# 3dlg-hcvc/tricolo

Measured on AMD Instinct MI355X. Metric: trimodal training samples/sec (32^3 voxel + 6-view), higher is better.
Workload: dtype f16 (f16 activation storage + f16 MFMA operands, fp32 accumulate; bf16x3 heads/GRU; within 1e-3 of the fp32 reference)

## Files before the change

include/tricolo_hip.h:

```cpp
#ifndef TRICOLO_HIP_H
#define TRICOLO_HIP_H
#include <stddef.h>
#include <stdint.h>

#ifdef __cplusplus
extern "C" {
#endif

#define TRI_FMT_F32 0
#define TRI_FMT_BF16 1
#define TRI_FMT_F16 2

int tri_version(void);
const char* tri_last_error(void);

typedef struct TriConvDesc {
    int B, ID, IH, IW, Cin;
    int OD, OH, OW, Cout;
    int KD, KH, KW, stride, pad_d, pad_h, pad_w;
} TriConvDesc;

int tri_conv_kpad(int ntaps, int cin_stored);
typedef struct TriPrepDesc {
    const float* w;
// ... 150 lines not shown
                        const float* mean, const float* invstd, float* dgamma, float* dbeta, float* c1, float* c2, float* c3,
                        float out_scale ,
                        void* stream);
int tri_bn_bwd_apply(const void* y, const void* g, const float* c1, const float* c2, const float* c3, const uint8_t* row_mask,
                     void* dy, long M, int C, const float* relu_scale, const float* relu_shift, const void* relu_out,
                     void* g_masked ,
                     int keep_inactive ,
                     int act_fmt, void* stream);
int tri_bn_bwd_pair_reduce(const void* ya, const void* yb, const void* g, const void* relu_out, long M, int C, float* partial_a,
                           float* partial_b, int act_fmt, void* stream);
int tri_bn_bwd_pair_finalize(const float* partial_a, const float* partial_b, int nblk, int C, int count_host, const float* gamma_a,
                             const float* mean_a, const float* invstd_a, float* buf_a, const float* gamma_b, const float* mean_b,
                             const float* invstd_b, float* buf_b, float out_scale, void* stream);
int tri_bn_bwd_pair_apply(const void* ya, const void* yb, const void* g, const void* relu_out, const float* buf_a, const float* buf_b,
                          void* dya, void* dyb, void* g_masked, long M, int C, int act_fmt, void* stream);

int tri_bn_relu_pool3d_fwd(const void* y, const float* scale, const float* shift, const uint8_t* mask, int B, int D, int C,
                           void* pooled, uint8_t* mask_out, int act_fmt, void* stream);
int tri_pool3d_bwd_route_rows(const void* y, const float* scale, const float* shift, const uint8_t* mask, const void* pooled,
                              const void* dpooled, int B, int D, int C, void* g, const int* out_pos, const int* out_count, int act_fmt,
                              void* stream);
int tri_pool3d_bwd_route_rows_num_blocks(int B, int D, int C);
int tri_pool3d_bwd_route_rows_reduce(const void* y, const float* scale, const float* shift, const uint8_t* mask, const void* pooled,
                                     const void* dpooled, int B, int D, int C, void* g, const int* out_pos, const int* out_count,
                                     float* partial, int act_fmt, void* stream);
int tri_bn_bwd_apply_rows(const void* y, const void* g, const float* c1, const float* c2, const float* c3, void* dy, int C,
                          const int* row_pos, const int* row_count, long max_rows, int act_fmt, void* stream);
size_t tri_bn_bwd_rows_scratch(int C);
int tri_bn_bwd_rows(const void* y, const void* g, int C, const int* row_pos, const int* row_count, long max_rows, const float* gamma,
                    const float* mean, const float* invstd, void* dy, float* dgamma, float* dbeta, float out_scale, void* scratch,
// ... 141 lines not shown
```

tricolo_amd/_C.py:

```python
from __future__ import annotations

import ctypes as C
import os

import torch

_HERE = os.path.dirname(os.path.abspath(__file__))
LIB_PATH = os.path.join(_HERE, "libtricolo_hip.so")


class TriConvDesc(C.Structure):
    _fields_ = [(n, C.c_int) for n in ("B", "ID", "IH", "IW", "Cin", "OD", "OH", "OW", "Cout",
                                       "KD", "KH", "KW", "stride", "pad_d", "pad_h", "pad_w")]


class TriPrepDesc(C.Structure):
    _fields_ = [("w", C.c_void_p), ("hi", C.c_void_p), ("lo", C.c_void_p), ("s_row", C.c_long), ("s_tap", C.c_long),
                ("s_inner", C.c_long), ("rows", C.c_int), ("ntaps", C.c_int), ("inner", C.c_int), ("inner_pad", C.c_int),
                ("kpad", C.c_int), ("fmt", C.c_int), ("frag", C.c_int)]


class TriWgradReduce(C.Structure):
    _fields_ = [("slab", C.c_void_p), ("dw", C.c_void_p), ("s_co", C.c_long), ("s_tap", C.c_long), ("s_ci", C.c_long)] + \
               [(n, C.c_int) for n in ("splits", "Cout", "Kpad", "ntaps", "cin_stored", "cin_real", "zlanes", "nblocks")] + \
# ... 57 lines not shown
    "tri_conv_stem_wgrad_bn": (I, [DP, P, P, P, P, P, P, P, P, P, P, Z, P, L, L, L, I, I, F, P, P]),
    "tri_conv_wgrad_group_info": (I, [DP, I, P, P, P]),
    "tri_conv_wgrad_partial_group": (I, [P, I, I, P, P]),
    "tri_bn_finalize": (I, [P, I, I, P, I, P, P, P, P, P, F, F, P, P, P, P, P]),
    "tri_bn_eval_coeffs": (I, [I, P, P, P, P, F, P, P, P, P, P]),
    "tri_bn_act": (I, [P, P, P, P, P, P, P, L, I, I, I, P]),
    "tri_relu_bwd": (I, [P, P, P, L, I, P]),
    "tri_bn_bwd_num_blocks": (I, [L]),
    "tri_bn_bwd_reduce": (I, [P, P, L, I, P, P, P, P, P, I, P]),
    "tri_bn_bwd_finalize": (I, [P, I, I, P, I, P, P, P, P, P, P, P, P, F, P]),
    "tri_bn_bwd_small": (I, [P, P, L, I, P, I, P, P, P, P, P, P, P, P, I, P, P, P, F, I, P]),
    "tri_bn_bwd_apply": (I, [P, P, P, P, P, P, P, L, I, P, P, P, P, I, I, P]),
    "tri_bn_bwd_pair_reduce": (I, [P, P, P, P, L, I, P, P, I, P]),
    "tri_bn_bwd_pair_finalize": (I, [P, P, I, I, I, P, P, P, P, P, P, P, P, F, P]),
    "tri_bn_bwd_pair_apply": (I, [P, P, P, P, P, P, P, P, P, L, I, I, P]),
    "tri_bn_relu_pool3d_fwd": (I, [P, P, P, P, I, I, I, P, P, I, P]),
    "tri_pool3d_bwd_route": (I, [P, P, P, P, P, P, I, I, I, P, I, P]),
    "tri_pool3d_bwd_route_rows": (I, [P, P, P, P, P, P, I, I, I, P, P, P, I, P]),
    "tri_pool3d_bwd_route_rows_num_blocks": (I, [I, I, I]),
    "tri_pool3d_bwd_route_rows_reduce": (I, [P, P, P, P, P, P, I, I, I, P, P, P, P, I, P]),
    "tri_bn_bwd_apply_rows": (I, [P, P, P, P, P, P, I, P, P, L, I, P]),
    "tri_bn_bwd_rows_scratch": (C.c_size_t, [I]),
    "tri_bn_bwd_rows": (I, [P, P, I, P, P, L, P, P, P, P, P, P, F, P, I, P]),
    "tri_pool3d_bwd_route_reduce_num_blocks": (I, [I, I, I]),
    "tri_pool3d_bwd_route_reduce": (I, [P, P, P, P, P, P, I, I, I, P, P, I, P]),
    "tri_maxpool2d_fwd": (I, [P, I, I, I, I, P, P, P, P, I, P]),
    "tri_maxpool2d_bwd": (I, [P, P, I, I, I, I, P, I, P]),
    "tri_maxpool_bn_bwd_num_blocks": (I, [I, I, I]),
    "tri_maxpool_bn_bwd_reduce": (I, [P, P, P, I, I, I, I, P, P, P, I, P]),
    "tri_maxpool_bn_bwd_pooled_num_blocks": (I, [I, I, I]),
# ... 138 lines not shown
```

tricolo_amd/csrc/bn_pool.hip:

```cpp
#include "common.h"
#include "../../include/tricolo_hip.h"

__global__ void bn_finalize_kernel(const float* __restrict__ partial, int ntiles, int C, const int* __restrict__ count_dev,
                                   int count_host, const float* __restrict__ gamma, const float* __restrict__ beta,
                                   float* running_mean, float* running_var, long long* num_batches_tracked, float momentum,
                                   float eps, float* __restrict__ mean_out, float* __restrict__ invstd_out,
                                   float* __restrict__ scale_out, float* __restrict__ shift_out) {
    __shared__ double ssum[4], ssq[4];
    const int c = blockIdx.x;
    float pg = 0.f, pb = 0.f, prm = 0.f, prv = 0.f;
    int pcount = count_host;
    if (threadIdx.x == 0) {
        pg = gamma[c]; pb = beta[c];
        if (running_mean) { prm = running_mean[c]; prv = running_var[c]; }
        if (count_dev) pcount = *count_dev;
    }
    double s = 0.0, q = 0.0;
#pragma unroll 8
    for (int tIdx = threadIdx.x; tIdx < ntiles; tIdx += 256) {
        s += (double)partial[((size_t)tIdx * 2 + 0) * C + c];
        q += (double)partial[((size_t)tIdx * 2 + 1) * C + c];
    }
#pragma unroll
    for (int o = 32; o > 0; o >>= 1) { s += __shfl_xor(s, o); q += __shfl_xor(q, o); }
// ... 162 lines not shown
    if (relu_scale && relu_out) { tri_set_error("tri_bn_bwd_reduce: give either relu_scale/shift or relu_out"); return TRI_ERR_ARG; }
#define TRI_BNR(MASK_)                                                                                                              \
    do {                                                                                                                            \
        if (row_mask) TRI_ACT_DISPATCH(act_fmt, bn_bwd_reduce_kernel<T, MASK_, true><<<nblk, 256, smem, (hipStream_t)stream>>>(       \
            (const T*)y, (const T*)g, M, C, partial, rows, (const float4*)relu_scale, (const float4*)relu_shift, (const T*)relu_out, row_mask)); \
        else TRI_ACT_DISPATCH(act_fmt, bn_bwd_reduce_kernel<T, MASK_, false><<<nblk, 256, smem, (hipStream_t)stream>>>(               \
            (const T*)y, (const T*)g, M, C, partial, rows, (const float4*)relu_scale, (const float4*)relu_shift, (const T*)relu_out, row_mask)); \
    } while (0)
    if (relu_out) TRI_BNR(2);
    else if (relu_scale) TRI_BNR(1);
    else TRI_BNR(0);
#undef TRI_BNR
    return tri_check_launch("tri_bn_bwd_reduce");
}

__device__ __forceinline__ void bn_bwd_finalize_body(const float* __restrict__ partial, int nblk, int C, const int* __restrict__ count_dev,
                                                     int count_host, const float* __restrict__ gamma, const float* __restrict__ mean,
                                                     const float* __restrict__ invstd, float* __restrict__ dgamma, float* __restrict__ dbeta,
                                                     float* __restrict__ c1, float* __restrict__ c2, float* __restrict__ c3, float out_scale,
                                                     int c) {
    __shared__ double ssum[4], ssq[4];
    float pmu = 0.f, pis = 0.f, pga = 0.f;
    int pcount = count_host;
    if (threadIdx.x == 0) {
        pmu = mean[c]; pis = invstd[c]; pga = gamma[c];
        if (count_dev) pcount = *count_dev;
    }
    double s = 0.0, q = 0.0;
#pragma unroll 8
    for (int b = threadIdx.x; b < nblk; b += 256) {
        s += (double)partial[((size_t)b * 2 + 0) * C + c];
        q += (double)partial[((size_t)b * 2 + 1) * C + c];
    }
#pragma unroll
    for (int o = 32; o > 0; o >>= 1) { s += __shfl_xor(s, o); q += __shfl_xor(q, o); }
    if ((threadIdx.x & 63) == 0) { ssum[threadIdx.x >> 6] = s; ssq[threadIdx.x >> 6] = q; }
    __syncthreads();
    if (threadIdx.x == 0) {
        s = (ssum[0] + ssum[1]) + (ssum[2] + ssum[3]);
        q = (ssq[0] + ssq[1]) + (ssq[2] + ssq[3]);
        double n = (double)pcount;
        if (n < 1.0) { dgamma[c] = 0.f; dbeta[c] = 0.f; c1[c] = 0.f; c2[c] = 0.f; c3[c] = 0.f; return; }
        double mu = pmu, is = pis, ga = pga;
        double dbe = s;
        double dga = is * (q - mu * s);
        dgamma[c] = (float)(dga * (double)out_scale);
        dbeta[c] = (float)(dbe * (double)out_scale);
        double k1 = ga * is;
        double k3 = -ga * is * is * dga / n;
        double k2 = -k1 * dbe / n - k3 * mu;
        c1[c] = (float)k1; c2[c] = (float)k2; c3[c] = (float)k3;
    }
}
__global__ void bn_bwd_finalize_kernel(const float* __restrict__ partial, int nblk, int C, const int* __restrict__ count_dev,
                                       int count_host, const float* __restrict__ gamma, const float* __restrict__ mean,
                                       const float* __restrict__ invstd, float* __restrict__ dgamma, float* __restrict__ dbeta,
                                       float* __restrict__ c1, float* __restrict__ c2, float* __restrict__ c3, float out_scale) {
    bn_bwd_finalize_body(partial, nblk, C, count_dev, count_host, gamma, mean, invstd, dgamma, dbeta, c1, c2, c3, out_scale, blockIdx.x);
}
__global__ void bn_bwd_finalize_pair_kernel(const float* __restrict__ pa, const float* __restrict__ pb, int nblk, int C, int count_host,
                                            const float* __restrict__ ga, const float* __restrict__ ma, const float* __restrict__ ia,
                                            float* __restrict__ buf_a, const float* __restrict__ gb, const float* __restrict__ mb,
                                            const float* __restrict__ ib, float* __restrict__ buf_b, float out_scale) {
    const bool second = (int)blockIdx.x >= C;
    const int c = second ? blockIdx.x - C : blockIdx.x;
    float* buf = second ? buf_b : buf_a;
// ... 139 lines not shown
                                        const float* invstd_b, float* buf_b, float out_scale, void* stream) {
    bn_bwd_finalize_pair_kernel<<<2 * C, 256, 0, (hipStream_t)stream>>>(partial_a, partial_b, nblk, C, count_host, gamma_a, mean_a, invstd_a, buf_a,
                                                                       gamma_b, mean_b, invstd_b, buf_b, out_scale);
    return tri_check_launch("tri_bn_bwd_pair_finalize");
}
extern "C" int tri_bn_bwd_pair_apply(const void* ya, const void* yb, const void* g, const void* relu_out, const float* buf_a, const float* buf_b,
                                     void* dya, void* dyb, void* g_masked, long M, int C, int act_fmt, void* stream) {
    if (C % 4) { tri_set_error("tri_bn_bwd_pair_apply: C must be a multiple of 4"); return TRI_ERR_ARG; }
    const long total4 = M * (C / 4);
    TRI_ACT_DISPATCH(act_fmt, bn_bwd_apply_pair_kernel<T><<<ew_grid(total4), 256, 0, (hipStream_t)stream>>>(
        (const T*)ya, (const T*)yb, (const T*)g, (const float4*)(buf_a + 2 * C), (const float4*)(buf_b + 2 * C), (T*)dya, (T*)dyb, total4, C / 4,
        (const T*)relu_out, (T*)g_masked));
    return tri_check_launch("tri_bn_bwd_pair_apply");
}

template <typename T, int MASK, int CH>
__global__ __launch_bounds__(256) void bn_bwd_small_kernel(const T* __restrict__ y, const T* g, long M, int C, const int* __restrict__ count_dev,
                                                           int count_host, const float* __restrict__ gamma, const float* __restrict__ mean,
                                                           const float* __restrict__ invstd, const float* __restrict__ rs,
                                                           const float* __restrict__ rb, const T* __restrict__ ro, T* gm,
                                                           const uint8_t* __restrict__ row_mask, int keep_inactive, T* dy,
                                                           float* __restrict__ dgamma, float* __restrict__ dbeta, float out_scale) {
    constexpr int Q = CH / 4;
    __shared__ float red[4][2 * CH];
    __shared__ float coef[3 * CH];
    const int nblk = gridDim.x;
    const int grp = (nblk % 8 == 0) ? (int)(blockIdx.x % 8) * (nblk / 8) + (int)(blockIdx.x / 8) : (int)blockIdx.x;
    const int c0 = grp * CH;
    const int t = threadIdx.x;
    float4 s4[Q], b4[Q];
// ... 1015 lines not shown
```

tricolo_amd/model/module/img_encoder/mv_cnn.py:

```python
from __future__ import annotations

import contextlib
import os

import torch
import torch.nn as nn

from .... import ops
from ....layers import SideStream, TriModule, linear_bwd, linear_fwd, require_gpu


_DS_FWD = int(os.environ.get("TRICOLO_DS_FWD", "2"))
_DS_BWD = int(os.environ.get("TRICOLO_DS_BWD", "2"))
_PREP_DGRAD_LATE = os.environ.get("TRICOLO_PREP_DGRAD_LATE", "1") != "0"
_BN_PAIR = True
_STEM_BESIDE_WGRAD = os.environ.get("TRICOLO_STEM_BESIDE_WGRAD", "1") != "0"
_PREP_ISSUE = int(os.environ.get("TRICOLO_PREP_ISSUE", "1"))


class _BasicBlockParams(nn.Module):
    def __init__(self, inplanes, planes, stride):
        super().__init__()
        self.conv1 = nn.Conv2d(inplanes, planes, 3, stride, 1, bias=False)
        self.bn1 = nn.BatchNorm2d(planes)
# ... 261 lines not shown
                gr[w] = ops.conv_wgrad(x, dy, g, w, prec, out_scale=ugs, batch=batch)
                return
            with torch.cuda.stream(side.fork(x, dy)):
                gr[w] = ops.conv_wgrad(x, dy, g, w, prec, out_scale=ugs)

        dout_sums = None
        for bi in range(len(blocks) - 1, -1, -1):
            blk, sv = blocks[bi], saved_blocks[bi]
            x, y1, co1, g1, a1, y2, co2, g2, yd, cod, gd, out = sv
            pair = (_BN_PAIR and blk.downsample is not None and batch is not None and dout_sums is None and yd is not None
                    and yd.shape == y2.shape and ops._sync_world() == 1)
            dyd_pair = None
            if pair:
                (dy2, gr[blk.bn2.weight], gr[blk.bn2.bias], dyd_pair, gr[blk.downsample[1].weight],
                 gr[blk.downsample[1].bias]) = ops.bn_bwd_pair(y2, co2, blk.bn2.weight, yd, cod, blk.downsample[1].weight, dout, out, g2.M,
                                                               g_masked=dout, out_scale=ugs)
            else:
                dy2, gr[blk.bn2.weight], gr[blk.bn2.bias] = ops.bn_bwd(y2, dout, co2, blk.bn2.weight, count_host=g2.M, inplace=False,
                                                                       relu_out=out, g_masked=dout, out_scale=ugs, partial=dout_sums)
            g = dout
            fine = ops.TIMELINE is not None and ops.TIMELINE.get("fine")
            tag = f"image.bwd.c{y2.shape[-1]}.b{bi}"
            if fine:
                ops.stamp(tag + ".bn2")
            mode = _DS_BWD if (blk.downsample is not None and batch is not None) else 0
            ev = None
            if mode == 2:
                ev = torch.cuda.Event()
                ev.record()

            def shortcut_bwd():
                with torch.cuda.stream(self._side_ds.fork(g, yd, event=ev)):
                    if dyd_pair is not None:
                        return dyd_pair, ops.conv_dgrad(dyd_pair, gd, self._packed[(id(blk.downsample[0]), True)])
                    dyd_, gr[blk.downsample[1].weight], gr[blk.downsample[1].bias] = ops.bn_bwd(
                        yd, g, cod, blk.downsample[1].weight, count_host=gd.M, inplace=False, out_scale=ugs)
                    if batch is None:
                        gr[blk.downsample[0].weight] = ops.conv_wgrad(x, dyd_, gd, blk.downsample[0].weight, prec, out_scale=ugs)
                    return dyd_, ops.conv_dgrad(dyd_, gd, self._packed[(id(blk.downsample[0]), True)])
            if blk.downsample is not None and not mode:
                dyd, dx = shortcut_bwd()
            wgrad_async(a1, dy2, g2, blk.conv2.weight)
            da1, sums1 = ops.conv_dgrad(dy2, g2, self._packed[(id(blk.conv2), True)], bn_sums=(y1, co1, None))
            if mode:
                dyd, dx = shortcut_bwd()
            if fine:
                ops.stamp(tag + ".dgrad2")
            dy1, gr[blk.bn1.weight], gr[blk.bn1.bias] = ops.bn_bwd(y1, da1, co1, blk.bn1.weight, count_host=g1.M, relu=True, out_scale=ugs,
                                                                   partial=sums1)
            if fine:
                ops.stamp(tag + ".bn1")
            wgrad_async(x, dy1, g1, blk.conv1.weight)
            if blk.downsample is not None:
                if batch is None:
                    self._side_ds.join(dx, gr[blk.downsample[0].weight], gr[blk.downsample[1].weight], gr[blk.downsample[1].bias])
                else:
                    self._side_ds.join(dx, dyd, gr[blk.downsample[1].weight], gr[blk.downsample[1].bias])
                    gr[blk.downsample[0].weight] = ops.conv_wgrad(x, dyd, gd, blk.downsample[0].weight, prec, out_scale=ugs, batch=batch)
            else:
                dx = g
            if bi > 0:
                prev = saved_blocks[bi - 1]
                dx, dout_sums = ops.conv_dgrad(dy1, g1, self._packed[(id(blk.conv1), True)], out=dx, accumulate=True,
                                               bn_sums=(prev[5], None, prev[11]))
# ... 122 lines not shown
```

tricolo_amd/ops.py:

```python
from __future__ import annotations

import collections
import math
import os

import torch

from . import _C
from ._C import check, lib, make_desc, ptr, stream

_PRECISIONS = ("bf16", "bf16x3", "f16")
_FMT = {torch.float32: 0, torch.bfloat16: 1, torch.float16: 2}
F16_GRAD_SCALE = float(os.environ.get("TRICOLO_F16_GRAD_SCALE", "4096"))
if not (F16_GRAD_SCALE >= 1.0 and math.frexp(F16_GRAD_SCALE)[0] == 0.5):
    raise ValueError(f"TRICOLO_F16_GRAD_SCALE={F16_GRAD_SCALE!r}: must be a power of two >= 1 (the kernels divide it out exactly)")
_default_precision = os.environ.get("TRICOLO_PRECISION", "bf16x3")


def set_default_precision(p: str):
    global _default_precision
    if p not in _PRECISIONS:
        raise ValueError(f"precision must be one of {_PRECISIONS}")
    _default_precision = p

# ... 660 lines not shown
        tot = _sync_sum(partial.sum(0, keepdim=True).contiguous())
        if count_dev is not None:
            count_dev = _sync_sum(count_dev.clone())
        else:
            count_host = int(count_host) * world
        gbuf = torch.empty((5, C), dtype=torch.float32, device=partial.device)
        check(lib().tri_bn_bwd_finalize(ptr(tot), 1, C, ptr(count_dev), int(count_host), ptr(gamma), ptr(co.mean), ptr(co.invstd), ptr(gbuf[0]),
                                        ptr(gbuf[1]), ptr(gbuf[2]), ptr(gbuf[3]), ptr(gbuf[4]), float(out_scale), stream()), "tri_bn_bwd_finalize")
        buf = torch.stack([buf[0], buf[1], gbuf[2], gbuf[3], gbuf[4]])
    return buf


_BN_SMALL = True


def _bn_bwd_finish(y, g, partial, co: BNCoeffs, gamma, count_dev, count_host, out_scale, dy, row_mask=None, keep_inactive=False, rows=None,
                   rs=None, rb=None, relu_out=None, g_masked=None):
    C = y.shape[-1]
    buf = _bn_bwd_finalize(partial, partial.shape[0], C, count_dev, count_host, gamma, co, out_scale)
    if rows is not None:
        check(lib().tri_bn_bwd_apply_rows(ptr(y), ptr(g), ptr(buf[2]), ptr(buf[3]), ptr(buf[4]), ptr(dy), C, ptr(rows[0]), ptr(rows[1]),
                                          rows[0].numel(), _abf(y), stream()), "tri_bn_bwd_apply_rows")
    else:
        check(lib().tri_bn_bwd_apply(ptr(y), ptr(g), ptr(buf[2]), ptr(buf[3]), ptr(buf[4]), ptr(row_mask), ptr(dy), y.numel() // C, C, ptr(rs), ptr(rb),
                                     ptr(relu_out), ptr(g_masked), 1 if keep_inactive else 0, _abf(y), stream()), "tri_bn_bwd_apply")
    return dy, buf[0], buf[1]


def bn_bwd(y, g, co: BNCoeffs, gamma, count_dev=None, count_host=0, row_mask=None, inplace=True, relu=False, relu_out=None,
           g_masked=None, out_scale: float = 1.0, keep_inactive: bool = False, partial=None):
    rs, rb = (co.scale, co.shift) if relu else (None, None)
    C = y.shape[-1]
    M = y.numel() // C
    assert y.dtype == g.dtype
    dy = g if inplace else torch.empty_like(g)
    if partial is None and _BN_SMALL and M <= 512 and C % 8 == 0 and C >= 64 and _sync_world() == 1:
        buf = torch.empty((2, C), dtype=torch.float32, device=y.device)
        check(lib().tri_bn_bwd_small(ptr(_act(y)), ptr(_act(g)), M, C, ptr(count_dev), int(count_host), ptr(gamma), ptr(co.mean), ptr(co.invstd),
                                     ptr(rs), ptr(rb), ptr(relu_out), ptr(g_masked), ptr(row_mask), 1 if keep_inactive else 0, ptr(dy), ptr(buf[0]),
                                     ptr(buf[1]), float(out_scale), _abf(y), stream()), "tri_bn_bwd_small")
        return dy, buf[0], buf[1]
    if partial is None:
        partial = torch.empty((lib().tri_bn_bwd_num_blocks(M), 2, C), dtype=torch.float32, device=y.device)
        check(lib().tri_bn_bwd_reduce(ptr(_act(y)), ptr(_act(g)), M, C, ptr(partial), ptr(rs), ptr(rb), ptr(relu_out), ptr(row_mask), _abf(y), stream()),
              "tri_bn_bwd_reduce")
    assert partial.shape[1:] == (2, C)
    return _bn_bwd_finish(y, g, partial, co, gamma, count_dev, count_host, out_scale, dy, row_mask=row_mask, keep_inactive=keep_inactive,
                          rs=rs, rb=rb, relu_out=relu_out, g_masked=g_masked)


def bn_bwd_pair(ya, coa: BNCoeffs, gamma_a, yb, cob: BNCoeffs, gamma_b, g, relu_out, count_host, g_masked=None, out_scale: float = 1.0):
    C = ya.shape[-1]
    M = ya.numel() // C
    assert ya.dtype == g.dtype == yb.dtype == relu_out.dtype and ya.shape == yb.shape and _sync_world() == 1
    nblk = lib().tri_bn_bwd_num_blocks(M)
    partial = torch.empty((2, nblk, 2, C), dtype=torch.float32, device=ya.device)
    check(lib().tri_bn_bwd_pair_reduce(ptr(_act(ya)), ptr(_act(yb)), ptr(_act(g)), ptr(relu_out), M, C, ptr(partial[0]), ptr(partial[1]), _abf(ya),
                                       stream()), "tri_bn_bwd_pair_reduce")
    buf = torch.empty((2, 5, C), dtype=torch.float32, device=ya.device)
    check(lib().tri_bn_bwd_pair_finalize(ptr(partial[0]), ptr(partial[1]), nblk, C, int(count_host), ptr(gamma_a), ptr(coa.mean), ptr(coa.invstd),
                                         ptr(buf[0]), ptr(gamma_b), ptr(cob.mean), ptr(cob.invstd), ptr(buf[1]), float(out_scale), stream()),
          "tri_bn_bwd_pair_finalize")
    dya, dyb = torch.empty_like(ya), torch.empty_like(yb)
    check(lib().tri_bn_bwd_pair_apply(ptr(ya), ptr(yb), ptr(g), ptr(relu_out), ptr(buf[0]), ptr(buf[1]), ptr(dya), ptr(dyb), ptr(g_masked), M, C,
                                      _abf(ya), stream()), "tri_bn_bwd_pair_apply")
    return dya, buf[0, 0], buf[0, 1], dyb, buf[1, 0], buf[1, 1]


def bn_relu_pool3d_fwd(y, co: BNCoeffs, mask, B, D, C, want_mask: bool = True):
# ... 957 lines not shown
```

Baseline: 13150.

## Fuse BN backward finalize into apply for a two-launch path in image encoder

Adds a two-launch BN backward path. A column-tiled reduce (centred on a bf16-rounded mean) is followed by an apply kernel that rebuilds the per-channel coefficients from the partial records in every workgroup, so the separate finalize launch goes away. The image encoder's residual blocks opt into it for the pair, single and relu-masked BN backward calls when M is at most 16384. Each apply workgroup now re-reduces up to 192 records, which adds redundant work in exchange for one fewer launch and no finalize round trip.

```diff
diff --git a/include/tricolo_hip.h b/include/tricolo_hip.h
--- a/include/tricolo_hip.h
+++ b/include/tricolo_hip.h
@@ -188,6 +188,21 @@
                              const float* invstd_b, float* buf_b, float out_scale, void* stream);
 int tri_bn_bwd_pair_apply(const void* ya, const void* yb, const void* g, const void* relu_out, const float* buf_a, const float* buf_b,
                           void* dya, void* dyb, void* g_masked, long M, int C, int act_fmt, void* stream);
+int tri_bnbwd2_records(long M, int C);
+int tri_bnbwd2_max_records(void);
+int tri_bnbwd2_reduce(const void* y, const void* g, long M, int C, float* partial, const float* relu_scale, const float* relu_shift,
+                      const void* relu_out, const float* mean , int act_fmt, void* stream);
+int tri_bnbwd2_apply(const void* y, const void* g, const float* partial, int nrec,
+                     int centred ,
+                     long M, int C, int count_host, const float* gamma, const float* mean, const float* invstd, float* dgamma, float* dbeta,
+                     float out_scale, const float* relu_scale, const float* relu_shift, const void* relu_out, void* g_masked, void* dy,
+                     int act_fmt, void* stream);
+int tri_bnbwd2_pair_reduce(const void* ya, const void* yb, const void* g, const void* relu_out, long M, int C, float* partial_a,
+                           float* partial_b, const float* mean_a, const float* mean_b, int act_fmt, void* stream);
+int tri_bnbwd2_pair_apply(const void* ya, const void* yb, const void* g, const void* relu_out, const float* partial_a,
+                          const float* partial_b, int nrec, long M, int C, int count_host, const float* gamma_a, const float* mean_a,
+                          const float* invstd_a, float* buf_a, const float* gamma_b, const float* mean_b, const float* invstd_b,
+                          float* buf_b, float out_scale, void* dya, void* dyb, void* g_masked, int act_fmt, void* stream);
 
 int tri_bn_relu_pool3d_fwd(const void* y, const float* scale, const float* shift, const uint8_t* mask, int B, int D, int C,
                            void* pooled, uint8_t* mask_out, int act_fmt, void* stream);
diff --git a/tricolo_amd/_C.py b/tricolo_amd/_C.py
--- a/tricolo_amd/_C.py
+++ b/tricolo_amd/_C.py
@@ -95,6 +95,12 @@
     "tri_bn_bwd_pair_reduce": (I, [P, P, P, P, L, I, P, P, I, P]),
     "tri_bn_bwd_pair_finalize": (I, [P, P, I, I, I, P, P, P, P, P, P, P, P, F, P]),
     "tri_bn_bwd_pair_apply": (I, [P, P, P, P, P, P, P, P, P, L, I, I, P]),
+    "tri_bnbwd2_records": (I, [L, I]),
+    "tri_bnbwd2_max_records": (I, []),
+    "tri_bnbwd2_reduce": (I, [P, P, L, I, P, P, P, P, P, I, P]),
+    "tri_bnbwd2_apply": (I, [P, P, P, I, I, L, I, I, P, P, P, P, P, F, P, P, P, P, P, I, P]),
+    "tri_bnbwd2_pair_reduce": (I, [P, P, P, P, L, I, P, P, P, P, I, P]),
+    "tri_bnbwd2_pair_apply": (I, [P, P, P, P, P, P, I, L, I, I, P, P, P, P, P, P, P, P, F, P, P, P, I, P]),
     "tri_bn_relu_pool3d_fwd": (I, [P, P, P, P, I, I, I, P, P, I, P]),
     "tri_pool3d_bwd_route": (I, [P, P, P, P, P, P, I, I, I, P, I, P]),
     "tri_pool3d_bwd_route_rows": (I, [P, P, P, P, P, P, I, I, I, P, P, P, I, P]),
diff --git a/tricolo_amd/csrc/bn_pool.hip b/tricolo_amd/csrc/bn_pool.hip
--- a/tricolo_amd/csrc/bn_pool.hip
+++ b/tricolo_amd/csrc/bn_pool.hip
@@ -200,6 +200,19 @@
     return tri_check_launch("tri_bn_bwd_reduce");
 }
 
+struct BnBwdCoeffs { float dgamma, dbeta, c1, c2, c3; };
+__device__ __forceinline__ BnBwdCoeffs bn_bwd_coeffs(double s, double q, double n, double mu, double is, double ga, float out_scale) {
+    BnBwdCoeffs r;
+    double dbe = s;
+    double dga = is * (q - mu * s);
+    r.dgamma = (float)(dga * (double)out_scale);
+    r.dbeta = (float)(dbe * (double)out_scale);
+    double k1 = ga * is;
+    double k3 = -ga * is * is * dga / n;
+    double k2 = -k1 * dbe / n - k3 * mu;
+    r.c1 = (float)k1; r.c2 = (float)k2; r.c3 = (float)k3;
+    return r;
+}
 __device__ __forceinline__ void bn_bwd_finalize_body(const float* __restrict__ partial, int nblk, int C, const int* __restrict__ count_dev,
                                                      int count_host, const float* __restrict__ gamma, const float* __restrict__ mean,
                                                      const float* __restrict__ invstd, float* __restrict__ dgamma, float* __restrict__ dbeta,
@@ -227,15 +240,9 @@
         q = (ssq[0] + ssq[1]) + (ssq[2] + ssq[3]);
         double n = (double)pcount;
         if (n < 1.0) { dgamma[c] = 0.f; dbeta[c] = 0.f; c1[c] = 0.f; c2[c] = 0.f; c3[c] = 0.f; return; }
-        double mu = pmu, is = pis, ga = pga;
-        double dbe = s;
-        double dga = is * (q - mu * s);
-        dgamma[c] = (float)(dga * (double)out_scale);
-        dbeta[c] = (float)(dbe * (double)out_scale);
-        double k1 = ga * is;
-        double k3 = -ga * is * is * dga / n;
-        double k2 = -k1 * dbe / n - k3 * mu;
-        c1[c] = (float)k1; c2[c] = (float)k2; c3[c] = (float)k3;
+        const BnBwdCoeffs k = bn_bwd_coeffs(s, q, n, pmu, pis, pga, out_scale);
+        dgamma[c] = k.dgamma; dbeta[c] = k.dbeta;
+        c1[c] = k.c1; c2[c] = k.c2; c3[c] = k.c3;
     }
 }
 __global__ void bn_bwd_finalize_kernel(const float* __restrict__ partial, int nblk, int C, const int* __restrict__ count_dev,
@@ -405,6 +412,308 @@
     return tri_check_launch("tri_bn_bwd_pair_apply");
 }
 
+static const int BN2_CH = 64;
+static const int BN2_RECORDS = 192;
+static const int BN2_APPLY_WGS = 768;
+struct Bn2Plan { long rows; int chunks; };
+static inline Bn2Plan bn2_plan(long M, int C, int wgs) {
+    long want = wgs / (C / BN2_CH);
+    if (want < 1) want = 1;
+    long rows = ((M + want - 1) / want + 15) / 16 * 16;
+    if (rows < 16) rows = 16;
+    Bn2Plan p;
+    p.rows = rows; p.chunks = (int)((M + rows - 1) / rows);
+    return p;
+}
+static int bn2_args_ok(long M, int C) {
+    if (M < 1 || C < BN2_CH || C % BN2_CH) { tri_set_error("tri_bnbwd2_*: needs M >= 1 rows and C a multiple of 64"); return 0; }
+    return 1;
+}
+template <int MASK>
+__device__ __forceinline__ float4 bn2_masked(float4 gv, const float4& yv, const float4& s4, const float4& b4, const float4& ov) {
+    if (MASK == 1) {
+        gv.x = __fmaf_rn(yv.x, s4.x, b4.x) > 0.f ? gv.x : 0.f; gv.y = __fmaf_rn(yv.y, s4.y, b4.y) > 0.f ? gv.y : 0.f;
+        gv.z = __fmaf_rn(yv.z, s4.z, b4.z) > 0.f ? gv.z : 0.f; gv.w = __fmaf_rn(yv.w, s4.w, b4.w) > 0.f ? gv.w : 0.f;
+    }
+    if (MASK == 2) { gv.x = ov.x > 0.f ? gv.x : 0.f; gv.y = ov.y > 0.f ? gv.y : 0.f; gv.z = ov.z > 0.f ? gv.z : 0.f; gv.w = ov.w > 0.f ? gv.w : 0.f; }
+    return gv;
+}
+__device__ __forceinline__ double bn2_sum16(const double* v) {
+    return (((v[0] + v[1]) + (v[2] + v[3])) + ((v[4] + v[5]) + (v[6] + v[7]))) + (((v[8] + v[9]) + (v[10] + v[11])) + ((v[12] + v[13]) + (v[14] + v[15])));
+}
+__device__ __forceinline__ float bn2_centre(float mean) { return (float)(bf16_t)mean; }
+template <typename T, int MASK>
+__global__ __launch_bounds__(256) void bn2_reduce_kernel(const T* __restrict__ y, const T* __restrict__ g, long M, int C, float* __restrict__ partial,
+                                                         long rows, const float4* __restrict__ rs, const float4* __restrict__ rb,
+                                                         const T* __restrict__ ro, const float4* __restrict__ mu) {
+    __shared__ double sh[16][16][8];
+    const int tc = threadIdx.x & 15, tr = threadIdx.x >> 4;
+    const int c4 = blockIdx.y * 16 + tc;
+    const long r0 = (long)blockIdx.x * rows;
+    const long r1 = r0 + rows < M ? r0 + rows : M;
+    double a[8] = {0, 0, 0, 0, 0, 0, 0, 0};
+    float4 s4 = make_float4(0, 0, 0, 0), b4 = make_float4(1, 1, 1, 1);
+    if (MASK == 1) { s4 = rs[c4]; b4 = rb[c4]; }
+    float4 m4 = make_float4(0, 0, 0, 0);
+    if (mu) { m4 = mu[c4]; m4 = make_float4(bn2_centre(m4.x), bn2_centre(m4.y), bn2_centre(m4.z), bn2_centre(m4.w)); }
+#pragma unroll 8
+    for (long r = r0 + tr; r < r1; r += 16) {
+        const long o = r * C + c4 * 4;
+        const float4 yv = Act<T>::ld4(y + o);
+        float4 ov = make_float4(0, 0, 0, 0);
+        if (MASK == 2) ov = Act<T>::ld4(ro + o);
+        const float4 gv = bn2_masked<MASK>(Act<T>::ld4(g + o), yv, s4, b4, ov);
+        a[0] += (double)gv.x; a[1] += (double)gv.y; a[2] += (double)gv.z; a[3] += (double)gv.w;
+        a[4] = fma((double)gv.x, (double)yv.x - (double)m4.x, a[4]); a[5] = fma((double)gv.y, (double)yv.y - (double)m4.y, a[5]);
+        a[6] = fma((double)gv.z, (double)yv.z - (double)m4.z, a[6]); a[7] = fma((double)gv.w, (double)yv.w - (double)m4.w, a[7]);
+    }
+    double* p = sh[tr][tc];
+#pragma unroll
+    for (int k = 0; k < 8; ++k) p[k] = a[k];
+    __syncthreads();
+    if (threadIdx.x < 128) {
+        const int half = threadIdx.x >> 6, ch = threadIdx.x & 63;
+        double v[16];
+#pragma unroll
+        for (int rr = 0; rr < 16; ++rr) v[rr] = sh[rr][ch >> 2][half * 4 + (ch & 3)];
+        partial[((size_t)blockIdx.x * 2 + half) * C + blockIdx.y * BN2_CH + ch] = (float)bn2_sum16(v);
+    }
+}
+__device__ __forceinline__ void bn2_coeffs(const float* __restrict__ partial, int nrec, int C, int c0, int count_host,
+                                           const float* __restrict__ gamma, const float* __restrict__ mean, const float* __restrict__ invstd,
+                                           float out_scale, bool centred, bool write, float* __restrict__ dgamma, float* __restrict__ dbeta,
+                                           double (*red)[128], float* coef) {
+    const int t = threadIdx.x;
+    float pmu = 0.f, pis = 0.f, pga = 0.f;
+    if (t < BN2_CH) { pmu = mean[c0 + t]; pis = invstd[c0 + t]; pga = gamma[c0 + t]; }
+    const int q = t & 31, lane = t >> 5;
+    const float* p = partial + (size_t)(q >> 4) * C + c0 + (q & 15) * 4;
+    double s0 = 0.0, s1 = 0.0, s2 = 0.0, s3 = 0.0;
+#pragma unroll 8
+    for (int b = lane; b < nrec; b += 8) {
+        const float4 v = *(const float4*)(p + (size_t)b * 2 * C);
+        s0 += (double)v.x; s1 += (double)v.y; s2 += (double)v.z; s3 += (double)v.w;
+    }
+    red[lane][q * 4 + 0] = s0; red[lane][q * 4 + 1] = s1; red[lane][q * 4 + 2] = s2; red[lane][q * 4 + 3] = s3;
+    __syncthreads();
+    if (t < BN2_CH) {
+        const double s = ((red[0][t] + red[1][t]) + (red[2][t] + red[3][t])) + ((red[4][t] + red[5][t]) + (red[6][t] + red[7][t]));
+        double sq = ((red[0][64 + t] + red[1][64 + t]) + (red[2][64 + t] + red[3][64 + t])) +
+                    ((red[4][64 + t] + red[5][64 + t]) + (red[6][64 + t] + red[7][64 + t]));
+        if (centred) sq = fma((double)bn2_centre(pmu), s, sq);
+        const double n = (double)count_host;
+        BnBwdCoeffs k = {0.f, 0.f, 0.f, 0.f, 0.f};
+        if (n >= 1.0) k = bn_bwd_coeffs(s, sq, n, pmu, pis, pga, out_scale);
+        coef[t] = k.c1; coef[BN2_CH + t] = k.c2; coef[2 * BN2_CH + t] = k.c3;
+        if (write) { dgamma[c0 + t] = k.dgamma; dbeta[c0 + t] = k.dbeta; }
+    }
+    __syncthreads();
+}
+template <typename T>
+__device__ __forceinline__ void bn2_store_twice(T* p, const float4& d, const float4& y, const float4& t) {
+    float4 o;
+    o.x = fp32_rounded(__fmaf_rn(d.x, y.x, t.x)); o.y = fp32_rounded(__fmaf_rn(d.y, y.y, t.y));
+    o.z = fp32_rounded(__fmaf_rn(d.z, y.z, t.z)); o.w = fp32_rounded(__fmaf_rn(d.w, y.w, t.w));
+    Act<T>::st4(p, o);
+}
+template <typename T>
+__device__ __forceinline__ void bn2_store_once(T* p, const float4& d, const float4& y, const float4& t) { bn2_store_twice(p, d, y, t); }
+template <>
+__device__ __forceinline__ void bn2_store_once<f16_t>(f16_t* p, const float4& d, const float4& y, const float4& t) {
+#if defined(__HIP_DEVICE_COMPILE__)
+    uint2 w = make_uint2(0u, 0u);
+    asm("v_fma_mixlo_f16 %0, %1, %2, %3 op_sel_hi:[0,0,0]" : "+v"(w.x) : "v"(d.x), "v"(y.x), "v"(t.x));
+    asm("v_fma_mixhi_f16 %0, %1, %2, %3 op_sel_hi:[0,0,0]" : "+v"(w.x) : "v"(d.y), "v"(y.y), "v"(t.y));
+    asm("v_fma_mixlo_f16 %0, %1, %2, %3 op_sel_hi:[0,0,0]" : "+v"(w.y) : "v"(d.z), "v"(y.z), "v"(t.z));
+    asm("v_fma_mixhi_f16 %0, %1, %2, %3 op_sel_hi:[0,0,0]" : "+v"(w.y) : "v"(d.w), "v"(y.w), "v"(t.w));
+    *(uint2*)p = w;
+#endif
+}
+__device__ __forceinline__ float4 bn2_fma4(const float4& a, const float4& g, const float4& b) {
+    return make_float4(__fmaf_rn(a.x, g.x, b.x), __fmaf_rn(a.y, g.y, b.y), __fmaf_rn(a.z, g.z, b.z), __fmaf_rn(a.w, g.w, b.w));
+}
+static const int BN2_U = 4;
+template <typename T, int MASK>
+__global__ __launch_bounds__(256) void bn2_apply_kernel(const T* __restrict__ y, const T* g, const float* __restrict__ partial, int nrec, long M,
+                                                        int C, int count_host, const float* __restrict__ gamma, const float* __restrict__ mean,
+                                                        const float* __restrict__ invstd, float* __restrict__ dgamma, float* __restrict__ dbeta,
+                                                        float out_scale, int centred, long rows, const float4* __restrict__ rs,
+                                                        const float4* __restrict__ rb, const T* __restrict__ ro, T* gm, T* dy) {
+    __shared__ double red[8][128];
+    __shared__ __attribute__((aligned(16))) float coef[3 * BN2_CH];
+    const int c0 = blockIdx.y * BN2_CH;
+    const int tc = threadIdx.x & 15, tr = threadIdx.x >> 4;
+    float4 s4 = make_float4(0, 0, 0, 0), b4 = make_float4(1, 1, 1, 1);
+    if (MASK == 1) { s4 = rs[c0 / 4 + tc]; b4 = rb[c0 / 4 + tc]; }
+    bn2_coeffs(partial, nrec, C, c0, count_host, gamma, mean, invstd, out_scale, centred != 0, blockIdx.x == 0, dgamma, dbeta, red, coef);
+    const float4 a = ((const float4*)coef)[tc], b = ((const float4*)(coef + BN2_CH))[tc], d = ((const float4*)(coef + 2 * BN2_CH))[tc];
+    const long r0 = (long)blockIdx.x * rows;
+    const long r1 = r0 + rows < M ? r0 + rows : M;
+    for (long r = r0 + tr; r < r1; r += 16 * BN2_U) {
+        float4 yv[BN2_U], gv[BN2_U], ov[BN2_U];
+#pragma unroll
+        for (int u = 0; u < BN2_U; ++u) {
+            const long o = (r + 16 * u) * C + c0 + tc * 4;
+            ov[u] = make_float4(0, 0, 0, 0);
+            if (r + 16 * u < r1) {
+                yv[u] = Act<T>::ld4(y + o); gv[u] = Act<T>::ld4(g + o);
+                if (MASK == 2) ov[u] = Act<T>::ld4(ro + o);
+            }
+        }
+#pragma unroll
+        for (int u = 0; u < BN2_U; ++u) {
+            if (r + 16 * u >= r1) continue;
+            const long o = (r + 16 * u) * C + c0 + tc * 4;
+            const float4 gm4 = bn2_masked<MASK>(gv[u], yv[u], s4, b4, ov[u]);
+            if (MASK == 2 && gm) Act<T>::st4(gm + o, gm4);
+            if (MASK == 0) bn2_store_once(dy + o, d, yv[u], bn2_fma4(a, gm4, b));
+            else bn2_store_twice(dy + o, d, yv[u], bn2_fma4(a, gm4, b));
+        }
+    }
+}
+template <typename T>
+__global__ __launch_bounds__(256) void bn2_reduce_pair_kernel(const T* __restrict__ ya, const T* __restrict__ yb, const T* __restrict__ g, long M,
+                                                              int C, float* __restrict__ partial_a, float* __restrict__ partial_b, long rows,
+                                                              const T* __restrict__ ro, const float4* __restrict__ mua,
+                                                              const float4* __restrict__ mub) {
+    __shared__ double sh[16][16][12];
+    const int tc = threadIdx.x & 15, tr = threadIdx.x >> 4;
+    const int c4 = blockIdx.y * 16 + tc;
+    const long r0 = (long)blockIdx.x * rows;
+    const long r1 = r0 + rows < M ? r0 + rows : M;
+    double a[12] = {0, 0, 0, 0, 0, 0, 0, 0, 0, 0, 0, 0};
+    float4 ma = mua[c4], mb = mub[c4];
+    ma = make_float4(bn2_centre(ma.x), bn2_centre(ma.y), bn2_centre(ma.z), bn2_centre(ma.w));
+    mb = make_float4(bn2_centre(mb.x), bn2_centre(mb.y), bn2_centre(mb.z), bn2_centre(mb.w));
+#pragma unroll 4
+    for (long r = r0 + tr; r < r1; r += 16) {
+        const long o = r * C + c4 * 4;
+        float4 gv = Act<T>::ld4(g + o);
+        const float4 av = Act<T>::ld4(ya + o), bv = Act<T>::ld4(yb + o), ov = Act<T>::ld4(ro + o);
+        gv.x = ov.x > 0.f ? gv.x : 0.f; gv.y = ov.y > 0.f ? gv.y : 0.f; gv.z = ov.z > 0.f ? gv.z : 0.f; gv.w = ov.w > 0.f ? gv.w : 0.f;
+        a[0] += (double)gv.x; a[1] += (double)gv.y; a[2] += (double)gv.z; a[3] += (double)gv.w;
+        a[4] = fma((double)gv.x, (double)av.x - (double)ma.x, a[4]); a[5] = fma((double)gv.y, (double)av.y - (double)ma.y, a[5]);
+        a[6] = fma((double)gv.z, (double)av.z - (double)ma.z, a[6]); a[7] = fma((double)gv.w, (double)av.w - (double)ma.w, a[7]);
+        a[8] = fma((double)gv.x, (double)bv.x - (double)mb.x, a[8]); a[9] = fma((double)gv.y, (double)bv.y - (double)mb.y, a[9]);
+        a[10] = fma((double)gv.z, (double)bv.z - (double)mb.z, a[10]); a[11] = fma((double)gv.w, (double)bv.w - (double)mb.w, a[11]);
+    }
+    double* p = sh[tr][tc];
+#pragma unroll
+    for (int k = 0; k < 12; ++k) p[k] = a[k];
+    __syncthreads();
+    if (threadIdx.x < 192) {
+        const int which = threadIdx.x >> 6, ch = threadIdx.x & 63;
+        double v[16];
+#pragma unroll
+        for (int rr = 0; rr < 16; ++rr) v[rr] = sh[rr][ch >> 2][which * 4 + (ch & 3)];
+        const float a = (float)bn2_sum16(v);
+        const size_t rec = (size_t)blockIdx.x * 2 * C + blockIdx.y * BN2_CH + ch;
+        if (which == 0) { partial_a[rec] = a; partial_b[rec] = a; }
+        else if (which == 1) partial_a[rec + C] = a;
+        else partial_b[rec + C] = a;
+    }
+}
+template <typename T>
+__global__ __launch_bounds__(256) void bn2_apply_pair_kernel(const T* __restrict__ ya, const T* __restrict__ yb, const T* g,
+                                                             const float* __restrict__ partial_a, const float* __restrict__ partial_b, int nrec,
+                                                             long M, int C, int count_host, const float* __restrict__ ga,
+                                                             const float* __restrict__ ma, const float* __restrict__ ia, float* __restrict__ buf_a,
+                                                             const float* __restrict__ gb, const float* __restrict__ mb,
+                                                             const float* __restrict__ ib, float* __restrict__ buf_b, float out_scale, long rows,
+                                                             const T* __restrict__ ro, T* gm, T* dya, T* dyb) {
+    __shared__ double red[8][128];
+    __shared__ __attribute__((aligned(16))) float coef[2][3 * BN2_CH];
+    const int c0 = blockIdx.y * BN2_CH;
+    const int tc = threadIdx.x & 15, tr = threadIdx.x >> 4;
+    bn2_coeffs(partial_a, nrec, C, c0, count_host, ga, ma, ia, out_scale, true, blockIdx.x == 0, buf_a, buf_a + C, red, coef[0]);
+    bn2_coeffs(partial_b, nrec, C, c0, count_host, gb, mb, ib, out_scale, true, blockIdx.x == 0, buf_b, buf_b + C, red, coef[1]);
+    const float4 a1 = ((const float4*)coef[0])[tc], a2 = ((const float4*)(coef[0] + BN2_CH))[tc], a3 = ((const float4*)(coef[0] + 2 * BN2_CH))[tc];
+    const float4 b1 = ((const float4*)coef[1])[tc], b2 = ((const float4*)(coef[1] + BN2_CH))[tc], b3 = ((const float4*)(coef[1] + 2 * BN2_CH))[tc];
+    const long r0 = (long)blockIdx.x * rows;
+    const long r1 = r0 + rows < M ? r0 + rows : M;
+    constexpr int U = 2;
+    for (long r = r0 + tr; r < r1; r += 16 * U) {
+        float4 av[U], bv[U], gv[U], ov[U];
+#pragma unroll
+        for (int u = 0; u < U; ++u) {
+            const long o = (r + 16 * u) * C + c0 + tc * 4;
+            if (r + 16 * u < r1) { gv[u] = Act<T>::ld4(g + o); av[u] = Act<T>::ld4(ya + o); bv[u] = Act<T>::ld4(yb + o); ov[u] = Act<T>::ld4(ro + o); }
+        }
+#pragma unroll
+        for (int u = 0; u < U; ++u) {
+            if (r + 16 * u >= r1) continue;
+            const long o = (r + 16 * u) * C + c0 + tc * 4;
+            float4 m = gv[u];
+            m.x = ov[u].x > 0.f ? m.x : 0.f; m.y = ov[u].y > 0.f ? m.y : 0.f; m.z = ov[u].z > 0.f ? m.z : 0.f; m.w = ov[u].w > 0.f ? m.w : 0.f;
+            if (gm) Act<T>::st4(gm + o, m);
+            bn2_store_twice(dya + o, a3, av[u], bn2_fma4(a1, m, a2));
+            bn2_store_once(dyb + o, b3, bv[u], bn2_fma4(b1, m, b2));
+        }
+    }
+}
+extern "C" int tri_bnbwd2_records(long M, int C) {
+    if (M < 1 || C < BN2_CH || C % BN2_CH) return 0;
+    return bn2_plan(M, C, BN2_RECORDS).chunks;
+}
+extern "C" int tri_bnbwd2_max_records(void) { return BN2_RECORDS; }
+extern "C" int tri_bnbwd2_reduce(const void* y, const void* g, long M, int C, float* partial, const float* relu_scale, const float* relu_shift,
+                                 const void* relu_out, const float* mean, int act_fmt, void* stream) {
+    if (!bn2_args_ok(M, C)) return TRI_ERR_UNSUPPORTED;
+    if ((relu_scale && relu_out) || (!relu_scale != !relu_shift)) { tri_set_error("tri_bnbwd2_reduce: give relu_scale + relu_shift, or relu_out, or neither"); return TRI_ERR_ARG; }
+    const Bn2Plan pl = bn2_plan(M, C, BN2_RECORDS);
+    const dim3 grid(pl.chunks, C / BN2_CH);
+#define TRI_BN2R(MASK_)                                                                                                                 \
+    TRI_ACT_DISPATCH(act_fmt, bn2_reduce_kernel<T, MASK_><<<grid, 256, 0, (hipStream_t)stream>>>(                                      \
+        (const T*)y, (const T*)g, M, C, partial, pl.rows, (const float4*)relu_scale, (const float4*)relu_shift, (const T*)relu_out,  \
+        (const float4*)mean))
+    if (relu_out) TRI_BN2R(2);
+    else if (relu_scale) TRI_BN2R(1);
+    else TRI_BN2R(0);
+#undef TRI_BN2R
+    return tri_check_launch("tri_bnbwd2_reduce");
+}
+extern "C" int tri_bnbwd2_apply(const void* y, const void* g, const float* partial, int nrec, int centred, long M, int C, int count_host,
+                                const float* gamma, const float* mean, const float* invstd, float* dgamma, float* dbeta, float out_scale, const float* relu_scale,
+                                const float* relu_shift, const void* relu_out, void* g_masked, void* dy, int act_fmt, void* stream) {
+    if (!bn2_args_ok(M, C)) return TRI_ERR_UNSUPPORTED;
+    if (nrec < 1 || nrec > BN2_RECORDS) { tri_set_error("tri_bnbwd2_apply: 1 .. 192 records"); return TRI_ERR_UNSUPPORTED; }
+    if ((relu_scale && relu_out) || (!relu_scale != !relu_shift)) { tri_set_error("tri_bnbwd2_apply: give relu_scale + relu_shift, or relu_out, or neither"); return TRI_ERR_ARG; }
+    const Bn2Plan pl = bn2_plan(M, C, BN2_APPLY_WGS);
+    const dim3 grid(pl.chunks, C / BN2_CH);
+#define TRI_BN2A(MASK_)                                                                                                                 \
+    TRI_ACT_DISPATCH(act_fmt, bn2_apply_kernel<T, MASK_><<<grid, 256, 0, (hipStream_t)stream>>>(                                       \
+        (const T*)y, (const T*)g, partial, nrec, M, C, count_host, gamma, mean, invstd, dgamma, dbeta, out_scale, centred, pl.rows,     \
+        (const float4*)relu_scale, (const float4*)relu_shift, (const T*)relu_out, (T*)g_masked, (T*)dy))
+    if (relu_out) TRI_BN2A(2);
+    else if (relu_scale) TRI_BN2A(1);
+    else TRI_BN2A(0);
+#undef TRI_BN2A
+    return tri_check_launch("tri_bnbwd2_apply");
+}
+extern "C" int tri_bnbwd2_pair_reduce(const void* ya, const void* yb, const void* g, const void* relu_out, long M, int C, float* partial_a,
+                                      float* partial_b, const float* mean_a, const float* mean_b, int act_fmt, void* stream) {
+    if (!bn2_args_ok(M, C)) return TRI_ERR_UNSUPPORTED;
+    if (!relu_out || !mean_a || !mean_b) { tri_set_error("tri_bnbwd2_pair_reduce: the saved output and both means are required"); return TRI_ERR_ARG; }
+    const Bn2Plan pl = bn2_plan(M, C, BN2_RECORDS);
+    const dim3 grid(pl.chunks, C / BN2_CH);
+    TRI_ACT_DISPATCH(act_fmt, bn2_reduce_pair_kernel<T><<<grid, 256, 0, (hipStream_t)stream>>>(
+        (const T*)ya, (const T*)yb, (const T*)g, M, C, partial_a, partial_b, pl.rows, (const T*)relu_out, (const float4*)mean_a, (const float4*)mean_b));
+    return tri_check_launch("tri_bnbwd2_pair_reduce");
+}
+extern "C" int tri_bnbwd2_pair_apply(const void* ya, const void* yb, const void* g, const void* relu_out, const float* partial_a,
+                                     const float* partial_b, int nrec, long M, int C, int count_host, const float* gamma_a, const float* mean_a,
+                                     const float* invstd_a, float* buf_a, const float* gamma_b, const float* mean_b, const float* invstd_b,
+                                     float* buf_b, float out_scale, void* dya, void* dyb, void* g_masked, int act_fmt, void* stream) {
+    if (!bn2_args_ok(M, C)) return TRI_ERR_UNSUPPORTED;
+    if (nrec < 1 || nrec > BN2_RECORDS || !relu_out) { tri_set_error("tri_bnbwd2_pair_apply: 1 .. 192 records and the saved output"); return TRI_ERR_UNSUPPORTED; }
+    const Bn2Plan pl = bn2_plan(M, C, BN2_APPLY_WGS);
+    const dim3 grid(pl.chunks, C / BN2_CH);
+    TRI_ACT_DISPATCH(act_fmt, bn2_apply_pair_kernel<T><<<grid, 256, 0, (hipStream_t)stream>>>(
+        (const T*)ya, (const T*)yb, (const T*)g, partial_a, partial_b, nrec, M, C, count_host, gamma_a, mean_a, invstd_a, buf_a, gamma_b, mean_b,
+        invstd_b, buf_b, out_scale, pl.rows, (const T*)relu_out, (T*)g_masked, (T*)dya, (T*)dyb));
+    return tri_check_launch("tri_bnbwd2_pair_apply");
+}
+
 template <typename T, int MASK, int CH>
 __global__ __launch_bounds__(256) void bn_bwd_small_kernel(const T* __restrict__ y, const T* g, long M, int C, const int* __restrict__ count_dev,
                                                            int count_host, const float* __restrict__ gamma, const float* __restrict__ mean,
diff --git a/tricolo_amd/model/module/img_encoder/mv_cnn.py b/tricolo_amd/model/module/img_encoder/mv_cnn.py
--- a/tricolo_amd/model/module/img_encoder/mv_cnn.py
+++ b/tricolo_amd/model/module/img_encoder/mv_cnn.py
@@ -299,10 +299,10 @@
             if pair:
                 (dy2, gr[blk.bn2.weight], gr[blk.bn2.bias], dyd_pair, gr[blk.downsample[1].weight],
                  gr[blk.downsample[1].bias]) = ops.bn_bwd_pair(y2, co2, blk.bn2.weight, yd, cod, blk.downsample[1].weight, dout, out, g2.M,
-                                                               g_masked=dout, out_scale=ugs)
+                                                               g_masked=dout, out_scale=ugs, two_launch=True)
             else:
                 dy2, gr[blk.bn2.weight], gr[blk.bn2.bias] = ops.bn_bwd(y2, dout, co2, blk.bn2.weight, count_host=g2.M, inplace=False,
-                                                                       relu_out=out, g_masked=dout, out_scale=ugs, partial=dout_sums)
+                                                                       relu_out=out, g_masked=dout, out_scale=ugs, partial=dout_sums, two_launch=True)
             g = dout
             fine = ops.TIMELINE is not None and ops.TIMELINE.get("fine")
             tag = f"image.bwd.c{y2.shape[-1]}.b{bi}"
@@ -332,7 +332,7 @@
             if fine:
                 ops.stamp(tag + ".dgrad2")
             dy1, gr[blk.bn1.weight], gr[blk.bn1.bias] = ops.bn_bwd(y1, da1, co1, blk.bn1.weight, count_host=g1.M, relu=True, out_scale=ugs,
-                                                                   partial=sums1)
+                                                                   partial=sums1, two_launch=True)
             if fine:
                 ops.stamp(tag + ".bn1")
             wgrad_async(x, dy1, g1, blk.conv1.weight)
diff --git a/tricolo_amd/ops.py b/tricolo_amd/ops.py
--- a/tricolo_amd/ops.py
+++ b/tricolo_amd/ops.py
@@ -698,9 +698,24 @@
 _BN_SMALL = True
 
 
+_BN2_MAX_ROWS = 16384
+
+
+def _bn_bwd_two_launches(asked, M, C, nrec=None, count_dev=None, row_mask=None, rows=None) -> bool:
+    if not asked or row_mask is not None or rows is not None or count_dev is not None or C % 64 or M > _BN2_MAX_ROWS or _sync_world() != 1:
+        return False
+    return nrec is None or 1 <= nrec <= lib().tri_bnbwd2_max_records()
+
+
 def _bn_bwd_finish(y, g, partial, co: BNCoeffs, gamma, count_dev, count_host, out_scale, dy, row_mask=None, keep_inactive=False, rows=None,
-                   rs=None, rb=None, relu_out=None, g_masked=None):
+                   rs=None, rb=None, relu_out=None, g_masked=None, two_launch=False, centred=False):
     C = y.shape[-1]
+    if _bn_bwd_two_launches(two_launch, y.numel() // C, C, partial.shape[0], count_dev, row_mask, rows):
+        buf = torch.empty((2, C), dtype=torch.float32, device=partial.device)
+        check(lib().tri_bnbwd2_apply(ptr(y), ptr(g), ptr(partial), partial.shape[0], 1 if centred else 0, y.numel() // C, C, int(count_host), ptr(gamma), ptr(co.mean),
+                                     ptr(co.invstd), ptr(buf[0]), ptr(buf[1]), float(out_scale), ptr(rs), ptr(rb), ptr(relu_out), ptr(g_masked),
+                                     ptr(dy), _abf(y), stream()), "tri_bnbwd2_apply")
+        return dy, buf[0], buf[1]
     buf = _bn_bwd_finalize(partial, partial.shape[0], C, count_dev, count_host, gamma, co, out_scale)
     if rows is not None:
         check(lib().tri_bn_bwd_apply_rows(ptr(y), ptr(g), ptr(buf[2]), ptr(buf[3]), ptr(buf[4]), ptr(dy), C, ptr(rows[0]), ptr(rows[1]),
@@ -712,7 +727,7 @@
 
 
 def bn_bwd(y, g, co: BNCoeffs, gamma, count_dev=None, count_host=0, row_mask=None, inplace=True, relu=False, relu_out=None,
-           g_masked=None, out_scale: float = 1.0, keep_inactive: bool = False, partial=None):
+           g_masked=None, out_scale: float = 1.0, keep_inactive: bool = False, partial=None, two_launch: bool = False):
     rs, rb = (co.scale, co.shift) if relu else (None, None)
     C = y.shape[-1]
     M = y.numel() // C
@@ -724,19 +739,37 @@
                                      ptr(rs), ptr(rb), ptr(relu_out), ptr(g_masked), ptr(row_mask), 1 if keep_inactive else 0, ptr(dy), ptr(buf[0]),
                                      ptr(buf[1]), float(out_scale), _abf(y), stream()), "tri_bn_bwd_small")
         return dy, buf[0], buf[1]
-    if partial is None:
+    centred = False
+    if partial is None and _bn_bwd_two_launches(two_launch, M, C, None, count_dev, row_mask):
+        partial, centred = torch.empty((lib().tri_bnbwd2_records(M, C), 2, C), dtype=torch.float32, device=y.device), True
+        check(lib().tri_bnbwd2_reduce(ptr(_act(y)), ptr(_act(g)), M, C, ptr(partial), ptr(rs), ptr(rb), ptr(relu_out), ptr(co.mean), _abf(y), stream()),
+              "tri_bnbwd2_reduce")
+    elif partial is None:
         partial = torch.empty((lib().tri_bn_bwd_num_blocks(M), 2, C), dtype=torch.float32, device=y.device)
         check(lib().tri_bn_bwd_reduce(ptr(_act(y)), ptr(_act(g)), M, C, ptr(partial), ptr(rs), ptr(rb), ptr(relu_out), ptr(row_mask), _abf(y), stream()),
               "tri_bn_bwd_reduce")
     assert partial.shape[1:] == (2, C)
     return _bn_bwd_finish(y, g, partial, co, gamma, count_dev, count_host, out_scale, dy, row_mask=row_mask, keep_inactive=keep_inactive,
-                          rs=rs, rb=rb, relu_out=relu_out, g_masked=g_masked)
-
-
-def bn_bwd_pair(ya, coa: BNCoeffs, gamma_a, yb, cob: BNCoeffs, gamma_b, g, relu_out, count_host, g_masked=None, out_scale: float = 1.0):
+                          rs=rs, rb=rb, relu_out=relu_out, g_masked=g_masked, two_launch=two_launch, centred=centred)
+
+
+def bn_bwd_pair(ya, coa: BNCoeffs, gamma_a, yb, cob: BNCoeffs, gamma_b, g, relu_out, count_host, g_masked=None, out_scale: float = 1.0,
+                two_launch: bool = False):
     C = ya.shape[-1]
     M = ya.numel() // C
     assert ya.dtype == g.dtype == yb.dtype == relu_out.dtype and ya.shape == yb.shape and _sync_world() == 1
+    if _bn_bwd_two_launches(two_launch, M, C):
+        nrec = lib().tri_bnbwd2_records(M, C)
+        partial = torch.empty((2, nrec, 2, C), dtype=torch.float32, device=ya.device)
+        check(lib().tri_bnbwd2_pair_reduce(ptr(_act(ya)), ptr(_act(yb)), ptr(_act(g)), ptr(relu_out), M, C, ptr(partial[0]), ptr(partial[1]), ptr(coa.mean),
+                                           ptr(cob.mean), _abf(ya), stream()), "tri_bnbwd2_pair_reduce")
+        buf = torch.empty((2, 2, C), dtype=torch.float32, device=ya.device)
+        dya, dyb = torch.empty_like(ya), torch.empty_like(yb)
+        check(lib().tri_bnbwd2_pair_apply(ptr(ya), ptr(yb), ptr(g), ptr(relu_out), ptr(partial[0]), ptr(partial[1]), nrec, M, C, int(count_host),
+                                          ptr(gamma_a), ptr(coa.mean), ptr(coa.invstd), ptr(buf[0]), ptr(gamma_b), ptr(cob.mean), ptr(cob.invstd),
+                                          ptr(buf[1]), float(out_scale), ptr(dya), ptr(dyb), ptr(g_masked), _abf(ya), stream()),
+              "tri_bnbwd2_pair_apply")
+        return dya, buf[0, 0], buf[0, 1], dyb, buf[1, 0], buf[1, 1]
     nblk = lib().tri_bn_bwd_num_blocks(M)
     partial = torch.empty((2, nblk, 2, C), dtype=torch.float32, device=ya.device)
     check(lib().tri_bn_bwd_pair_reduce(ptr(_act(ya)), ptr(_act(yb)), ptr(_act(g)), ptr(relu_out), M, C, ptr(partial[0]), ptr(partial[1]), _abf(ya),
```

Result: no change. 13220, median of 6 (+0.5%).
